# haoxiangsnr/Wave-U-Net-for-Speech-Enhancement

Measured on AMD Instinct MI355X. Metric: 16384-sample frames/sec fwd+bwd, 12-level Wave-U-Net, higher is better.
Workload: dtype f32 (levels >= 16 samples: 3 x f16 MFMA on hi/lo fp16 halves, fp32 accumulate; the rest f32 MFMA); 1 GPU; unet_basic 12-level, 16384-sample frames, batch=64 per GPU, fp32, training-mode forward + smooth_l1 + backward + fused HIP Adam step (BASELINE.json configs[2]; configs[3] when n_gpus>1); global_batch=64, frame=16384, parallelism=dp1

## Files before the change

### wave-u-net-for-speech-enhancement_amd/csrc/wunet_backward.cpp

```cpp
#include "wunet_host.h"
#include "wunet_elementwise.h"
#include "wunet_tiny.h"
#include "wunet_h3_elem.h"
#include "wunet_input_grad.h"

using namespace wunet_host;

namespace {
#ifndef WUNET_EMU
__global__ void stamp_kernel(unsigned long long* p) { *p = wall_clock64(); }
unsigned long long* g_stamps = nullptr;
bool stamps_on()
{
    static const bool on = getenv("WUNET_STAMP") != nullptr;
    if (on && !g_stamps && (hipMalloc(&g_stamps, 128 * sizeof(unsigned long long)) != hipSuccess || hipMemset(g_stamps, 0, 128 * sizeof(unsigned long long)) != hipSuccess)) g_stamps = nullptr;
    return on && g_stamps;
}
#define WUNET_STAMP(stream_, slot_) { if (stamps_on()) hipLaunchKernelGGL(stamp_kernel, dim3(1), dim3(1), 0, stream_, g_stamps + (slot_)); }
#else
#define WUNET_STAMP(stream_, slot_) {}
#endif

bool dx_stays_split(const wunet_ctx* c, int i)
{
// ... 259 lines not shown
    }
    return q.dx_sum ? sum_dx_splits(k, l) : WUNET_OK;
}

int weight_gradient(const BwdCall& k, int i, const BwdLayerPlan& q)
{
    wunet_ctx* c = k.c; float* ws = k.ws; const hipStream_t sd = k.sd;
    const int NL = c->NL;
    const LayerPlan& l = c->ly[i];
    if (sd != k.st && hipStreamWaitEvent(sd, k.side->ev_fork, 0) != hipSuccess) return fail(WUNET_E_RUNTIME, "fork onto the weight-gradient stream failed");
    WUNET_STAMP(sd, 2 * i + 1)
    if (i == NL - 1) {
        WUNET_LAUNCH(rows_sum_kernel, dim3(2), dim3(WUNET_THREADS), 0, sd,
                     (const float*)(ws + c->hpart_off), c->head_blocks, 2, k.grads[4 * NL] + c->ci, 1, k.grads[4 * NL + 1]);
        WUNET_CHECK_LAUNCH();
        WUNET_LAUNCH(rows_sum_kernel, dim3(c->ci), dim3(WUNET_THREADS), 0, sd,
                     (const float*)(ws + c->hpart2_off), l.a_split, c->ci, k.grads[4 * NL], c->ci, k.grads[4 * NL + 1]);
        WUNET_CHECK_LAUNCH();
    }
    if (q.e0) return WUNET_OK;
    const float* xin = i == 0 ? k.noisy : ws + l.xin;
    const size_t nw = (size_t)l.cout * l.cin * l.taps;
    if (q.tiny) {
        WUNET_LAUNCH(tiny_wgrad_kernel, dim3((unsigned)((nw + WUNET_THREADS - 1) / WUNET_THREADS)), dim3(WUNET_THREADS), 0, sd,
                     (const float*)(ws + l.g), xin, k.grads[4 * i], c->B, l.cin, l.cout, l.L, l.taps);
        WUNET_CHECK_LAUNCH();
        return WUNET_OK;
    }
    int rc;
    if (l.h3w)
        rc = launch_wgrad_h3(l, l.hw, reinterpret_cast<const wunet_half*>(ws + l.xh), reinterpret_cast<const wunet_half*>(ws + l.xl),
                             reinterpret_cast<const wunet_half*>(ws + l.gzh), reinterpret_cast<const wunet_half*>(ws + l.gzl),
                             gz_scale_slot(c, ws, i), x_scale_slot(c, ws, i),
                             ws + c->wgpart_off, c->B, sd, c->bf);
    else {
        WgradArgs w = make_wgrad_args(xin, ws + l.g, ws + c->wgpart_off, c->B, l.cin, l.cout, l.L, l.taps, l.w.cps);
        if (q.gz_in_wgrad) {
            w.z = ws + l.z; w.k1 = ws + l.k1; w.k2 = ws + l.k2; w.k3 = ws + l.k3; w.Lt = l.Lt;
        }
        rc = launch_wgrad_any(l.taps, w, l.w, sd);
    }
    if (rc) return rc;
    WUNET_CHECK_LAUNCH();
    if (l.h3w) {
        WgradH3ReduceArgs ra{};
        ra.part = ws + c->wgpart_off; ra.part_stride = h3w_part_stride(l, l.hw); ra.splits = l.hw.ksplit; ra.dw = k.grads[4 * i];
        ra.Cout = l.cout; ra.Cin = l.cin; ra.taps = l.taps; ra.mrep = l.hw.mrep; ra.tw = l.taps == 15 ? 8 : 5;
        ra.nblocks = l.hw.nblocks; ra.mblocks = l.hw.mblocks; ra.cib = l.taps == 15 ? 32 : 64;
        int serial_max = 64; long long serial_min_n4 = 8192;
#ifdef WUNET_EMU
        if (const char* e = getenv("WUNET_REDUCE_SERIAL")) sscanf(e, "%d,%lld", &serial_max, &serial_min_n4);
#endif
        const size_t n4 = ra.part_stride / 4;
        if (ra.splits <= serial_max && (long long)n4 >= serial_min_n4) {
            WUNET_LAUNCH(wgrad_h3_reduce_serial_kernel, dim3(capped_blocks(n4, WUNET_THREADS, 4096)), dim3(WUNET_THREADS), 0, sd, ra);
        } else {
            WUNET_LAUNCH(wgrad_h3_reduce_kernel, dim3(capped_blocks(n4, 16, 4096)), dim3(WUNET_THREADS), 0, sd, ra);
        }
    } else {
        const unsigned blocks = capped_blocks(nw / 4, 16, 4096);
        WUNET_LAUNCH(wgrad_reduce_kernel, dim3(blocks < 1 ? 1 : blocks), dim3(WUNET_THREADS), 0, sd,
                     (const float*)(ws + c->wgpart_off), l.w.rows, nw, k.grads[4 * i]);
    }
    WUNET_CHECK_LAUNCH();
    return WUNET_OK;
}

// ... 123 lines not shown
```

### wave-u-net-for-speech-enhancement_amd/csrc/wunet_h3.h

```cpp
#pragma once
#include "wunet_dev.h"

#ifdef WUNET_EMU
static const unsigned wunet_zero16[8] = {0, 0, 0, 0, 0, 0, 0, 0};
#else
static __device__ __attribute__((aligned(16))) const unsigned wunet_zero16[8] = {0, 0, 0, 0, 0, 0, 0, 0};
#endif

struct ConvH3Args {
    const wunet_half* xh; const wunet_half* xl;
    const wunet_half* wh; const wunet_half* wl;
    unsigned xdelta, wdelta;
    const void* zpad;
    const float* bias;
    const float* sc;
    const float* sc2;
    float* out;
    float* stats;
    const float* ev_a; const float* ev_s; float* xrows;
    unsigned long long* trace;
    int B, Cout, C8, NCH, L, logL;
    int NS, NFS;
    int ntiles, mblocks;
    int stages_per_split;
// ... 134 lines not shown
                {
                    const int krow = ((ks * 32) / LSEG) * SWX + (ks * 32) % LSEG;
                    const wunet_half* p = xs + xbase + (krow + OB + tw) * 8;
                    const wunet_h8 bh = wunet_ldtr8(p, p + 32);
                    wunet_h8 bl = bh;
                    if (!BF) bl = wunet_ldtr8(p + XG * XPOS * 8, p + XG * XPOS * 8 + 32);
#pragma unroll
                    for (int mt = 0; mt < M_REP; ++mt) {
                        if (BF) acc[mt][tw] = wunet_mfma16b(ah[mt], bh, acc[mt][tw]);
                        else {
                            acc[mt][tw] = wunet_mfma16h(al[mt], bh, acc[mt][tw]);
                            acc[mt][tw] = wunet_mfma16h(ah[mt], bl, acc[mt][tw]);
                            acc[mt][tw] = wunet_mfma16h(ah[mt], bh, acc[mt][tw]);
                        }
                    }
                }
            }
        }
    }
#undef WUNET_WH3_PREFETCH

    WUNET_WH3_STORE_PART(M_REP, TW, A, acc, blockIdx.x, (size_t)blockIdx.z * gridDim.y + blockIdx.y, wave, lane)
}

struct WgradH3dArgs {
    const wunet_half* xh; const wunet_half* xl;
    const wunet_half* gh; const wunet_half* gl;
    const float* sc;
    const float* sc2;
    float* part;
    int B, Cin, Cout, XC8, GC8, L, logL, chunks_per_split;
    size_t part_stride;
    int cin_active;
    int xcd_walk, ksplit, nblocks, mblocks;
};

template <int TAPS, int M_REP, bool DB, bool BF = false, int TP = 128>
__global__ __launch_bounds__(WUNET_THREADS, ((DB && TP == 128) ? 1 : 2)) void wgrad_h3d_kernel(WgradH3dArgs A)
{
    constexpr int GP = TP + 4, XPOS = TP + 20;
    static_assert(TP == 128 || TP == 64, "chunk");
    constexpr int WG = TAPS == 15 ? 2 : 4;
    constexpr int TW = TAPS == 15 ? 8 : 5;
    constexpr int OB = TAPS == 15 ? 1 : 8 - TAPS / 2;
    constexpr int CIB = WG * 16, XG = CIB / 8, GG = M_REP * 2;
    constexpr int NPL = BF ? 1 : 2;
    constexpr int GPCS = NPL * GG * GP;
    constexpr int XPCS = NPL * XG * XPOS;
    constexpr int GIT = (GPCS + WUNET_THREADS - 1) / WUNET_THREADS;
    constexpr int XIT = (XPCS + WUNET_THREADS - 1) / WUNET_THREADS;
    constexpr int BUF = (GPCS + XPCS + 8) * 8;
    WUNET_DYN_SMEM(smem);
    wunet_half* lds = reinterpret_cast<wunet_half*>(smem);

    const int tid = threadIdx.x, lane = tid & 63, wave = tid >> 6, q = lane >> 4, i16 = lane & 15;
    const int grp = TAPS == 15 ? wave >> 1 : wave;
    const int t0 = TAPS == 15 ? (wave & 1) * 8 : 0;
    int bx = blockIdx.x, by = blockIdx.y, bz = blockIdx.z;
    if (A.xcd_walk) {
        const int nyz = A.nblocks * A.mblocks;
        const int grp8 = (int)blockIdx.x / (8 * nyz), rem = (int)blockIdx.x - grp8 * 8 * nyz;
        const int yz = rem >> 3;
        bx = grp8 * 8 + (rem & 7); by = yz % A.nblocks; bz = yz / A.nblocks;
        if (bx >= A.ksplit) return;
    }
    const int co0 = bz * M_REP * 16, ci0 = by * CIB;
    const int L = A.L;
    const long long nchunks = ((long long)A.B * L) / TP;
    const long long kbeg = (long long)bx * A.chunks_per_split;
    long long kend = kbeg + A.chunks_per_split;
    if (kend > nchunks) kend = nchunks;

    const int tr_row = (i16 >> 2) + q * 8, tr_pl = (i16 & 3) >> 1, tr_h = (i16 & 1) * 4;
    const int gbase = (tr_pl * GP + tr_row) * 8 + tr_h;
    const int xbase = GPCS * 8 + ((grp * 2 + tr_pl) * XPOS + tr_row + t0) * 8 + tr_h;

    long long gsrc[GIT]; int gsel[GIT];
    long long xsrc[XIT]; int xrow[XIT], xsel[XIT];
#pragma unroll
    for (int it = 0; it < GIT; ++it) {
        const int f = tid + it * WUNET_THREADS;
        const int pl = f / GP, r = f - pl * GP;
        const int c8 = (co0 >> 3) + (pl % GG);
        gsel[it] = (f < GPCS && r < TP) ? ((c8 < A.GC8 ? 1 : 0) | (pl >= GG ? 2 : 0)) : -1;
        gsrc[it] = ((long long)c8 * L + r) * 8;
    }
#pragma unroll
    for (int it = 0; it < XIT; ++it) {
        const int f = tid + it * WUNET_THREADS;
        const int pl = f / XPOS, r = f - pl * XPOS;
        const int c8 = (ci0 >> 3) + (pl % XG);
        xsel[it] = f < XPCS ? ((c8 < A.XC8 ? 1 : 0) | (pl >= XG ? 2 : 0)) : -1;
        xrow[it] = r - 8;
        xsrc[it] = ((long long)c8 * L + (r - 8)) * 8;
    }
    const wunet_half* const zero_ = reinterpret_cast<const wunet_half*>(wunet_zero16);
#define WUNET_WH3D_DMA(K_, BUF_)                                                                                  \
    {                                                                                                             \
        const long long n0_ = (K_) * TP;                                                                          \
        const int b_ = (int)(n0_ >> A.logL), l0_ = (int)(n0_ & (L - 1));                                          \
        wunet_half* dst_ = lds + (size_t)(BUF_) * BUF + (size_t)wave * 64 * 8;                                    \
        _Pragma("unroll") for (int it = 0; it < GIT; ++it) {                                                      \
            if (gsel[it] >= 0) {                                                                                  \
                const wunet_half* src_ = (gsel[it] & 2) ? A.gl : A.gh;                                            \
                const wunet_half* p_ = (gsel[it] & 1) ? src_ + (size_t)b_ * A.GC8 * L * 8 + gsrc[it] + (size_t)l0_ * 8 : zero_; \
                wunet_dma16(p_, dst_ + (size_t)it * WUNET_THREADS * 8);                                           \
            }                                                                                                     \
        }                                                                                                         \
        _Pragma("unroll") for (int it = 0; it < XIT; ++it) {                                                      \
            if (xsel[it] >= 0) {                                                                                  \
                const int l_ = l0_ + xrow[it];                                                                    \
                const wunet_half* src_ = (xsel[it] & 2) ? A.xl : A.xh;                                            \
                const wunet_half* p_ = ((xsel[it] & 1) && l_ >= 0 && l_ < L)                                      \
                                           ? src_ + (size_t)b_ * A.XC8 * L * 8 + xsrc[it] + (size_t)l0_ * 8 : zero_; \
                wunet_dma16(p_, dst_ + (size_t)GPCS * 8 + (size_t)it * WUNET_THREADS * 8);                        \
            }                                                                                                     \
        }                                                                                                         \
    }

    wunet_f4 acc[M_REP][TW];
#pragma unroll
    for (int mt = 0; mt < M_REP; ++mt)
#pragma unroll
        for (int tw = 0; tw < TW; ++tw) acc[mt][tw] = wunet_f4{0.f, 0.f, 0.f, 0.f};

    const bool active = wunet_uniform(ci0 + grp * 16 < A.cin_active ? 1 : 0) != 0;
    if (DB && kbeg < kend) WUNET_WH3D_DMA(kbeg, 0)
    for (long long k = kbeg; k < kend; ++k) {
        const int cur = DB ? (int)((k - kbeg) & 1) : 0;
        if (!DB) {
            __syncthreads();
            WUNET_WH3D_DMA(k, 0)
        }
        wunet_dma_wait();
        __syncthreads();
        if (DB && k + 1 < kend) WUNET_WH3D_DMA(k + 1, cur ^ 1)
        const wunet_half* gs = lds + (size_t)cur * BUF;
        constexpr int KS = TP / 32;
        if (!active) continue;
        wunet_h8 ah[2][M_REP], al[2][M_REP], bh[2], bl[2];
#define WUNET_WH3D_LOAD_A(BUF_, KS_)                                                                              \
    _Pragma("unroll") for (int mt = 0; mt < M_REP; ++mt) {                                                        \
        const wunet_half* p = gs + gbase + ((mt * 2) * GP + (KS_) * 32) * 8;                                      \
        ah[BUF_][mt] = wunet_ldtr8(p, p + 32);                                                                    \
        if (!BF) al[BUF_][mt] = wunet_ldtr8(p + GG * GP * 8, p + GG * GP * 8 + 32);                               \
    }
#define WUNET_WH3D_LOAD_B(BUF_, KS_, TW_)                                                                         \
    {                                                                                                             \
        const wunet_half* p = gs + xbase + ((KS_) * 32 + OB + (TW_)) * 8;                                         \
        bh[BUF_] = wunet_ldtr8(p, p + 32);                                                                        \
        if (!BF) bl[BUF_] = wunet_ldtr8(p + XG * XPOS * 8, p + XG * XPOS * 8 + 32);                               \
    }
        WUNET_WH3D_LOAD_A(0, 0)
        WUNET_WH3D_LOAD_B(0, 0, 0)
#pragma unroll
        for (int ks = 0; ks < KS; ++ks) {
#pragma unroll
            for (int tw = 0; tw < TW; ++tw) {
                const int sb = (ks * TW + tw) & 1, ab = ks & 1;
                if (tw + 1 < TW) {
                    if (sb) { WUNET_WH3D_LOAD_B(0, ks, tw + 1) } else { WUNET_WH3D_LOAD_B(1, ks, tw + 1) }
                } else if (ks + 1 < KS) {
                    if (ab) { WUNET_WH3D_LOAD_A(0, ks + 1) } else { WUNET_WH3D_LOAD_A(1, ks + 1) }
                    if (sb) { WUNET_WH3D_LOAD_B(0, ks + 1, 0) } else { WUNET_WH3D_LOAD_B(1, ks + 1, 0) }
                }
                wunet_sched_fence();
                if (BF) {
#pragma unroll
                    for (int mt = 0; mt < M_REP; ++mt) acc[mt][tw] = wunet_mfma16b(ah[ab][mt], bh[sb], acc[mt][tw]);
                } else {
#pragma unroll
                    for (int mt = 0; mt < M_REP; ++mt) acc[mt][tw] = wunet_mfma16h(al[ab][mt], bh[sb], acc[mt][tw]);
#pragma unroll
                    for (int mt = 0; mt < M_REP; ++mt) acc[mt][tw] = wunet_mfma16h(ah[ab][mt], bl[sb], acc[mt][tw]);
#pragma unroll
                    for (int mt = 0; mt < M_REP; ++mt) acc[mt][tw] = wunet_mfma16h(ah[ab][mt], bh[sb], acc[mt][tw]);
                }
            }
        }
#undef WUNET_WH3D_LOAD_A
#undef WUNET_WH3D_LOAD_B
    }
#undef WUNET_WH3D_DMA

    WUNET_WH3_STORE_PART(M_REP, TW, A, acc, bx, (size_t)bz * (A.xcd_walk ? (unsigned)A.nblocks : gridDim.y) + by, wave, lane)
}
```

### wave-u-net-for-speech-enhancement_amd/csrc/wunet_host.h

```cpp
#pragma once
#include <cstdarg>
#include <cmath>
#include <cstdio>
#include <cstdlib>
#include <cstring>
#include <map>
#include <mutex>
#include <string>
#include <vector>

#include "wunet_kernels.h"
#include "wunet_h3.h"
#include "wunet_h3u.h"
#include "wunet_launch.h"
#include "wunet_hip.h"

namespace wunet_host {

int fail(int code, const char* fmt, ...);
const char* last_error_text();

#define WUNET_CHECK_LAUNCH()                                                                   \
    do {                                                                                       \
        hipError_t e_ = hipGetLastError();                                                     \
        if (e_ != hipSuccess) return wunet_host::fail(WUNET_E_RUNTIME, "%s:%d HIP error: %s", __FILE__, __LINE__, hipGetErrorString(e_)); \
    } while (0)

extern bool g_prof_on;
void prof_begin(hipStream_t st, const char* name, double flops, double bytes);
void prof_end(hipStream_t st);
long long prof_collect(char* buf, size_t cap);
extern unsigned long long* g_h3_trace;

inline int ilog2(long long v) { int r = 0; while ((1LL << r) < v) ++r; return r; }
inline bool is_pow2(long long v) { return v > 0 && (v & (v - 1)) == 0; }
inline size_t align64(size_t v) { return (v + 63) & ~(size_t)63; }
inline int round_up(int v, int m) { return (v + m - 1) / m * m; }
inline unsigned capped_blocks(size_t n, size_t per_block, size_t cap) { const size_t b = (n + per_block - 1) / per_block; return (unsigned)(b < cap ? b : cap); }
inline int kc_of(int taps) { return taps == 15 ? 4 : 12; }

struct ConvCfg { int mrep, nrep, mtiles_p, mblocks, cp, grid_x, ksplit, kcps; };
ConvCfg plan_conv(int B, int L, int rows, int kch, int taps);
ConvArgs make_conv_args(const float* x, int kch, const float* wpk, const float* bias, float* out, float* stats,
                        int B, int rows, int L, int taps, const ConvCfg& c, size_t split_stride);
int launch_conv(int taps, const ConvArgs& a, const ConvCfg& c, hipStream_t st);

struct WgradCfg { int mrep, nw, xit, wsplit, mblocks, nblocks, ksplit, cps, rows; };
WgradCfg plan_wgrad(int B, int L, int cin, int cout, int taps);
WgradArgs make_wgrad_args(const float* x, const float* g, float* part, int B, int Cin, int Cout, int L, int taps, int cps);
int launch_wgrad_any(int taps, const WgradArgs& a, const WgradCfg& w, hipStream_t st);

enum { LK_RAW = 0, LK_DECIM = 1, LK_UPCAT = 2 };

struct PlanSwitches {
    const char *order_f, *order_d, *order_w;
    bool no_split, old_split, ktail_off, no_skip_fuse, no_evop, no_e0, upt_off, wgrad_xcd_off;
    int sps, h3u_eval, h3u_train, a_cap;
};
PlanSwitches read_plan_switches();

struct H3ConvPlan { int mrep, mtp, nch, sps, ksplit, ntiles, ntt; };
H3ConvPlan plan_h3_conv(int B, int L, int rows, int kch, int taps, bool transposed, int bf, const PlanSwitches& sw);
struct H3WgradPlan { int mrep, mblocks, nblocks, ksplit, cps, tp, xcd, dma, db; };
H3WgradPlan plan_h3_wgrad(int B, int L, int cin, int cout, int taps, int bf, const PlanSwitches& sw);

struct LayerGeom {
    int cin, cout, taps, L, logL, kind;
    int Lt;
    int src0, src1;
    int c0;
};
struct LayerDecisions {
    ConvCfg f;
    ConvCfg d;
    WgradCfg w;
    int f_rows;
    int a_split;
    size_t f_wpk, d_wpk;
    size_t z, a, s, mean, rstd, xin, g, dx, k1, k2, k3;
    size_t wl1;
    int evop;
    int h3f, h3d, h3w;
    H3ConvPlan hf, hd;
    H3WgradPlan hw;
    int first;
    int h3x;
    int skip_from;
    int h3u, h3u_train;
    int feeds_h3;
    size_t xh, xl, xzp;
    size_t gzh, gzl, gzp;
    size_t h3f_wpk, h3d_wpk;
    int upt;
    size_t dxh, usp;
};
struct LayerPlan : LayerGeom, LayerDecisions {};

size_t h3d_smem(int nseg, int mrep, int bf, int mtp, int eval, int upt = 0);
int h3d_blocks_per_cu(int nseg, int mrep, int bf);
int h3_stage_count(int kch, int taps, int ntt);
size_t h3w_part_stride(const LayerGeom& g, const H3WgradPlan& w);
size_t h3w_dma_smem(const LayerGeom& g, const H3WgradPlan& w, int bf);
bool up_pairs_regular(int Lin);
unsigned pack_gx();

}

struct wunet_ctx {
    int n, ci, B, T, NL;
    int Tt = 0;
    bool padded = false;
    size_t pad_in = 0, pad_out = 0, pad_gout = 0;
    std::vector<wunet_host::LayerPlan> ly;
    size_t stats_off, wpkf_off, spart_off, fwd_floats;
    size_t bmax_off, bound_off;
    size_t bpart_off, wgpart_off, wpkb_off, gh_off, hpart_off, hpart2_off, e0part_off, total_floats;
    int e0 = 1;
    int head_blocks;
    int h3 = 0;
    int bf = 0;
    std::vector<unsigned char> frozen;
    bool any_frozen = false;
    size_t h3_wf_hi, h3_wf_lo, h3_wb_hi, h3_wb_lo, h3_slot;
    size_t fslot_off, wmax_off;
    size_t h3_wf_halfs, h3_wb_halfs;
    struct Side {
        hipStream_t stream = nullptr; hipEvent_t ev_fork = nullptr, ev_join = nullptr, ev_pack = nullptr, ev_fpack = nullptr, ev_fpack2 = nullptr;
        const void* packed_ws = nullptr;
    };
    std::map<int, Side> side;
    std::mutex side_lock;
};

namespace wunet_host {

void layout_workspace(wunet_ctx* c);
int launch_split(const float* x, wunet_half* hi, wunet_half* lo, const float* sc, const float* xb0, const float* xb1, float* xsc,
                 int B, int C, int L, hipStream_t st, int bf = 0);
float* x_scale_slot(const wunet_ctx* c, float* ws, int layer);
float* w_scale_slot(const wunet_ctx* c, float* ws, int layer);
float* act_bound_slot(const wunet_ctx* c, float* ws, int layer);
float* gz_scale_slot(const wunet_ctx* c, float* ws, int layer);
struct ConvH3OpOut { wunet_half* h; wunet_half* l; const float* wl1; const float* xmax; float* xsc; int C8; };
struct ConvH3Upt { int c0; float up_scale; float* uh_out; float* uh_spill; };
struct ConvH3Launch {
    int taps, mrep, mtiles_p, sps, nch, ntt;
    int B, rows, kch, L, bf;
    const wunet_half *xh, *xl, *wh, *wl;
    const void* zpad;
    const float *bias, *sc, *sc2;
    float *out, *stats;
    const float *ev_a, *ev_s; float* xrows;
    const ConvH3OpOut* op;
    const ConvH3Upt* upt;
};
int launch_conv_h3(const ConvH3Launch& k, hipStream_t st);
int launch_conv_h3u(const ConvH3uArgs& a, int mrep, int mtiles_p, int kch, hipStream_t st);
int launch_wgrad_h3(const LayerGeom& g, const H3WgradPlan& w, const wunet_half* xh, const wunet_half* xl, const wunet_half* gh, const wunet_half* gl,
                    const float* sc, const float* sc2, float* part, int B, hipStream_t st, int bf = 0);
int launch_backward_packs(wunet_ctx* c, const float* const* params, float* ws, hipStream_t st);
wunet_ctx::Side* side_for_current_device(wunet_ctx* c);
bool side_stream_off();

}
```

### wave-u-net-for-speech-enhancement_amd/csrc/wunet_launchers.cpp

```cpp
#include "wunet_host.h"
#include "wunet_elementwise.h"
#include "wunet_h3_elem.h"

namespace wunet_host {

ConvArgs make_conv_args(const float* x, int kch, const float* wpk, const float* bias, float* out, float* stats,
                        int B, int rows, int L, int taps, const ConvCfg& c, size_t split_stride)
{
    ConvArgs a{};
    a.x = x; a.wpk = wpk; a.bias = bias; a.out = out; a.stats = stats;
    a.B = B; a.Cin = kch; a.Cout = rows; a.CinP = c.cp; a.L = L; a.logL = ilog2(L);
    const int tn = 64 * c.nrep;
    a.seg = L < tn ? L : tn;
    a.seg_shift = ilog2(a.seg);
    a.segw = a.seg + 16;
    const int rowlen = (tn / a.seg) * a.segw;
    int rp = rowlen;
    while (rp % 32 != 16) rp += 4;
    a.rowp = rp;
    a.r4 = rowlen / 4;
    a.sw4 = a.segw / 4;
    a.r4_magic = (unsigned)(((1u << 20) + a.r4 - 1) / a.r4);
    a.sw4_magic = (unsigned)(((1u << 20) + a.sw4 - 1) / a.sw4);
    a.kc_per_split = c.kcps;
// ... 121 lines not shown
    if (gx < nitems) gx &= ~7;
    if (gx < 8) gx = 8;
    if (gx > nitems) gx = nitems;
    const dim3 grid((unsigned)gx, (unsigned)ksplit);
    const int rc = wunet_launch_conv_h3d(a, taps, mrep, nseg, grid, smem, st, bf != 0, op != nullptr, upt != nullptr);
    prof_end(st);
    if (rc != 0) return fail(WUNET_E_ARG, "no conv_h3 kernel for taps=%d mrep=%d nseg=%d (rc %d)", taps, mrep, nseg, rc);
    return 0;
}

int launch_conv_h3u(const ConvH3uArgs& a0, int mrep, int mtiles_p, int kch, hipStream_t st)
{
    ConvH3uArgs a = a0;
    const double posn = (double)a.B * a.L;
    a.logL = ilog2(a.L);
    a.C8 = (kch + 7) / 8;
    a.NS = (a.C8 + 3) / 4;
    a.ntiles = (int)((posn + 255) / 256); a.mblocks = mtiles_p / mrep;
    a.trace = g_h3_trace ? g_h3_trace + (1 << 20) : nullptr;
    const size_t smem = (size_t)(2 * 2 * 4 * 272 + 2 * 2 * mrep * 5 * 64) * 16 + (size_t)(WUNET_WAVES * mrep * 32 + 4 + 2 * a.C8 * 8 + 3 * mtiles_p * 16) * sizeof(float);
    const int nitems = a.ntiles * a.mblocks;
    int gx = h3_grid_cap() / 2;
    if (gx > nitems) gx = nitems;
    char pname[64];
    snprintf(pname, sizeof pname, "conv_h3u_kernel<%d>", mrep);
    prof_begin(st, pname, 2.0 * posn * a.Cout * kch * 5.0, 4.0 * posn * (a.Cout + a.C0 * 0.5 + a.C1));
    const int rc = wunet_launch_conv_h3u(a, mrep, dim3((unsigned)gx), smem, st);
    prof_end(st);
    if (rc != 0) return fail(WUNET_E_ARG, "no conv_h3u kernel for mrep=%d (rc %d)", mrep, rc);
    return 0;
}

int launch_wgrad_h3(const LayerGeom& l, const H3WgradPlan& w, const wunet_half* xh, const wunet_half* xl, const wunet_half* gh, const wunet_half* gl,
                    const float* sc, const float* sc2, float* part, int B, hipStream_t st, int bf)
{
    char pname[96];
    const double posn = (double)B * l.L;
    const int xg = l.taps == 15 ? 4 : 8, tp = w.tp, nseg = l.L >= tp ? 1 : tp / l.L;
    const dim3 grid(w.ksplit, w.nblocks, w.mblocks);
    const int npl = bf ? 1 : 2;
    int rc;
    const auto fill = [&](auto& a) {
        a.xh = xh; a.xl = xl; a.gh = gh; a.gl = gl; a.sc = sc; a.sc2 = sc2; a.part = part; a.B = B; a.Cin = l.cin; a.Cout = l.cout;
        a.XC8 = (l.cin + 7) / 8; a.GC8 = (l.cout + 7) / 8; a.L = l.L; a.logL = l.logL;
        a.chunks_per_split = w.cps; a.part_stride = h3w_part_stride(l, w);
    };
    snprintf(pname, sizeof pname, "wgrad_h3%s_kernel<%d, %d%s>", w.dma ? "d" : "", l.taps, w.mrep, bf ? ", bf16" : "");
    prof_begin(st, pname, 2.0 * posn * l.cout * l.cin * l.taps, 4.0 * posn * (l.cout + l.cin));
    if (w.dma) {
        WgradH3dArgs a{};
        fill(a);
        a.cin_active = l.cin;
        a.ksplit = w.ksplit; a.nblocks = w.nblocks; a.mblocks = w.mblocks;
        a.xcd_walk = w.xcd;
        const size_t smem_d = h3w_dma_smem(l, w, bf);
        const int nyz = w.nblocks * w.mblocks;
        const dim3 grid_x((unsigned)(((w.ksplit + 7) / 8) * 8 * nyz));
        rc = wunet_launch_wgrad_h3d(a, l.taps, w.mrep, w.db != 0, a.xcd_walk ? grid_x : grid, w.db ? smem_d : smem_d / 2, st, bf != 0, tp);
    } else {
        WgradH3Args a{};
        fill(a);
        const int xrows = nseg == 1 ? tp + 20 : nseg * (tp / nseg + 16), xpos = ((xrows + 11) / 16) * 16 + 4;
        const size_t smem = ((size_t)npl * (w.mrep * 2) * (tp + 4) + (size_t)npl * xg * xpos + 8) * 16;
        rc = wunet_launch_wgrad_h3(a, l.taps, w.mrep, nseg, tp, grid, smem, st, bf != 0);
    }
    prof_end(st);
    if (rc != 0) return fail(WUNET_E_ARG, "no wgrad_h3 kernel for taps=%d mrep=%d (rc %d)", l.taps, w.mrep, rc);
    return 0;
}

int launch_backward_packs(wunet_ctx* c, const float* const* params, float* ws, hipStream_t st)
{
    const int NL = c->NL;
    PackTable tab{};
    int nd = 0;
    for (int i = 1; i < NL; ++i) {
        const LayerPlan& l = c->ly[i];
        if (l.h3d) continue;
        PackDesc& d = tab.d[nd++];
        d.w = params[4 * i]; d.dst = ws + c->wpkb_off + l.d_wpk;
        d.Cout = l.cout; d.Cin = l.cin; d.taps = l.taps; d.M = l.cin; d.CP = l.d.cp; d.mtiles = l.d.mtiles_p; d.transposed = 1;
    }
    if (nd > 0) {
        WUNET_LAUNCH(pack_weights_kernel, dim3(pack_gx(), nd), dim3(WUNET_THREADS), 0, st, tab);
        WUNET_CHECK_LAUNCH();
// ... 54 lines not shown
```

### wave-u-net-for-speech-enhancement_amd/csrc/wunet_ops.cpp

```cpp
#include "wunet_host.h"
#include "wunet_elementwise.h"
#include "wunet_h3_elem.h"
#include "wunet_loss_rows.h"
#include "wunet_stft.h"
#include "wunet_stoi.h"
#include "wunet_mix.h"
#include "wunet_reverb.h"

using namespace wunet_host;

extern "C" {

size_t wunet_loss_scratch_bytes(void) { return 256 * sizeof(double); }

int wunet_loss_forward(int kind, const float* clean, const float* enhanced, size_t n, float* loss_out, void* scratch, void* stream)
{
    if (kind < 0 || kind > 2 || !clean || !enhanced || !loss_out || !scratch || n == 0) return fail(WUNET_E_ARG, "bad loss argument");
    hipStream_t st = (hipStream_t)stream;
    const unsigned blocks = capped_blocks(n, WUNET_THREADS * 8, 256);
    WUNET_LAUNCH(loss_partial_kernel, dim3(blocks), dim3(WUNET_THREADS), 0, st, kind, clean, enhanced, n, (double*)scratch);
    WUNET_CHECK_LAUNCH();
    WUNET_LAUNCH(loss_final_kernel, dim3(1), dim3(WUNET_THREADS), 0, st, (const double*)scratch, (int)blocks, n, loss_out);
    WUNET_CHECK_LAUNCH();
    return WUNET_OK;
// ... 825 lines not shown
    ConvH3Launch h{};
    h.taps = K; h.mrep = p.mrep; h.mtiles_p = p.mtp; h.sps = p.sps; h.nch = p.nch; h.ntt = p.ntt;
    h.B = B; h.rows = rows; h.kch = kch; h.L = L;
    h.xh = xs.h(); h.xl = xs.l(); h.zpad = xs.zpad(); h.wh = whp; h.wl = wlp;
    h.bias = split ? nullptr : bias; h.sc = xslot; h.sc2 = wslot + 2; h.out = split ? part.f() : out;
    rc = launch_conv_h3(h, st);
    if (!rc && split) {
        const unsigned blocks = capped_blocks(nout, WUNET_THREADS, 2048);
        const float* partp = part.f();
        const int ks = p.ksplit;
        WUNET_LAUNCH(split_sum_kernel, dim3(blocks), dim3(WUNET_THREADS), 0, st, partp, ks, nout, out, bias, rows, ilog2(L));
    }
    hipStreamSynchronize(st);
    if (rc) return rc;
    WUNET_CHECK_LAUNCH();
    return WUNET_OK;
}
}

int wunet_op_conv1d_split(const float* x, const float* w, const float* bias, float* z, int B, int Cin, int Cout, int L, int K, void* stream)
{
    if (op_split_check(B, Cin, Cout, L, K, false)) return WUNET_E_ARG;
    return op_conv_split_common(x, w, bias, z, B, Cin, Cout, Cout, Cin, L, K, 0, (hipStream_t)stream);
}

int wunet_op_conv1d_dgrad_split(const float* gz, const float* w, float* dx, int B, int Cin, int Cout, int L, int K, void* stream)
{
    if (op_split_check(B, Cin, Cout, L, K, true)) return WUNET_E_ARG;
    return op_conv_split_common(gz, w, nullptr, dx, B, Cout, Cin, Cout, Cin, L, K, 1, (hipStream_t)stream);
}

int wunet_op_conv1d_wgrad_split(const float* gz, const float* x, float* dw, int B, int Cin, int Cout, int L, int K, void* stream)
{
    if (op_split_check(B, Cin, Cout, L, K, true)) return WUNET_E_ARG;
    hipStream_t st = (hipStream_t)stream;
    LayerGeom l{};
    l.cin = Cin; l.cout = Cout; l.taps = K; l.L = L; l.logL = ilog2(L);
    const H3WgradPlan w = plan_h3_wgrad(B, L, Cin, Cout, K, 0, read_plan_switches());
    SplitBuf xs, gs;
    DevBuf misc, part;
    const int cmax = Cin > Cout ? Cin : Cout;
    if (!misc.alloc((16 + 2 * (size_t)cmax) * sizeof(float)) || !part.alloc((size_t)w.ksplit * h3w_part_stride(l, w) * sizeof(float)))
        return fail(WUNET_E_RUNTIME, "hipMalloc");
    float* gslot = misc.f(), *xslot = misc.f() + 8, *oz = misc.f() + 16;
    WUNET_LAUNCH(fill_kernel, dim3(4), dim3(WUNET_THREADS), 0, st, oz, (size_t)cmax, 1.0f);
    WUNET_LAUNCH(fill_kernel, dim3(4), dim3(WUNET_THREADS), 0, st, oz + cmax, (size_t)cmax, 0.0f);
    int rc = op_split_operand(gz, B, Cout, L, gs, gslot, oz, oz + cmax, st);
    if (!rc) rc = op_split_operand(x, B, Cin, L, xs, xslot, oz, oz + cmax, st);
    if (!rc) rc = launch_wgrad_h3(l, w, xs.h(), xs.l(), gs.h(), gs.l(), gslot, xslot, part.f(), B, st);
    if (!rc) {
        WgradH3ReduceArgs ra{};
        ra.part = part.f(); ra.part_stride = h3w_part_stride(l, w); ra.splits = w.ksplit; ra.dw = dw;
        ra.Cout = Cout; ra.Cin = Cin; ra.taps = K; ra.mrep = w.mrep; ra.tw = K == 15 ? 8 : 5;
        ra.nblocks = w.nblocks; ra.mblocks = w.mblocks; ra.cib = K == 15 ? 32 : 64;
        WUNET_LAUNCH(wgrad_h3_reduce_kernel, dim3(capped_blocks(ra.part_stride / 4, 16, 4096)), dim3(WUNET_THREADS), 0, st, ra);
    }
    hipStreamSynchronize(st);
    if (rc) return rc;
    WUNET_CHECK_LAUNCH();
    return WUNET_OK;
}

}
```

### wave-u-net-for-speech-enhancement_amd/csrc/wunet_plan.cpp

```cpp
#include <algorithm>
#include "wunet_host.h"
#include "wunet_h3_elem.h"

namespace wunet_host {

namespace { thread_local std::string g_err; }

int fail(int code, const char* fmt, ...)
{
    char buf[512];
    va_list ap;
    va_start(ap, fmt);
    vsnprintf(buf, sizeof buf, fmt, ap);
    va_end(ap);
    g_err = buf;
    return code;
}

const char* last_error_text() { return g_err.c_str(); }

namespace {
struct ProfRec { std::string name; double flops; double bytes; hipEvent_t e0, e1; };
std::vector<ProfRec> g_prof;
}
// ... 151 lines not shown
        const int occ_lds = (int)(160 * 1024 / lds);
        if (occ_lds < occ) occ = occ_lds < 1 ? 1 : occ_lds;
        const long long slots = 256LL * occ;
        const long long mn = (long long)w.mblocks * w.nblocks;
        long long ks = slots / mn;
        if (ks < 1) ks = 1;
        if (ks > chunks) ks = chunks;
        w.ksplit = (int)ks;
        w.cps = (int)((chunks + ks - 1) / ks);
        w.ksplit = (int)((chunks + w.cps - 1) / w.cps);
    }
    w.rows = w.ksplit * (w.wsplit ? 4 : 1);
    return w;
}
unsigned pack_gx() { return 512; }

PlanSwitches read_plan_switches()
{
    const auto is_zero = [](const char* name) { const char* e = getenv(name); return e != nullptr && atoi(e) == 0; };
    PlanSwitches sw{};
    sw.order_f = getenv("WUNET_H3_ORDER"); sw.order_d = getenv("WUNET_H3D_ORDER"); sw.order_w = getenv("WUNET_H3W_ORDER");
    sw.no_split = getenv("WUNET_H3_NOSPLIT") != nullptr; sw.old_split = getenv("WUNET_H3_OLDSPLIT") != nullptr;
    if (const char* e = getenv("WUNET_H3_SPS")) sw.sps = atoi(e);
    sw.ktail_off = is_zero("WUNET_H3_KTAIL");
    sw.h3u_eval = 512; sw.h3u_train = 2048;
    if (const char* e = getenv("WUNET_H3U")) {
        int a = 0, b = 0;
        const int got = sscanf(e, "%d,%d", &a, &b);
        if (got == 2) { sw.h3u_eval = a; sw.h3u_train = b; }
        else if (got == 1) sw.h3u_eval = sw.h3u_train = a;
    }
    sw.no_skip_fuse = getenv("WUNET_NO_SKIP_FUSE") != nullptr; sw.no_evop = getenv("WUNET_NO_EVOP") != nullptr; sw.no_e0 = getenv("WUNET_NO_E0") != nullptr;
    sw.upt_off = is_zero("WUNET_UPT"); sw.wgrad_xcd_off = is_zero("WUNET_WGRAD_XCD");
    sw.a_cap = getenv("WUNET_A_CAP") ? atoi(getenv("WUNET_A_CAP")) : 128;
    return sw;
}

int pick_mrep_h3(int mtiles, const char* ord)
{
    int best = 2, best_pad = 1 << 30;
    for (const char* p = ord; *p; ++p) {
        const int m = *p - '0';
        const int pad = round_up(mtiles, m) - mtiles;
        if (pad < best_pad) { best_pad = pad; best = m; }
    }
    return best;
}

const char* h3_order(int taps, int L, int ntiles, int mtiles)
{
    return (taps == 5 && L >= 256 && (long long)ntiles * ((mtiles + 3) / 4) >= 512) ? "432" : "32";
}

size_t h3w_part_stride(const LayerGeom& g, const H3WgradPlan& w)
{
    const int tw = g.taps == 15 ? 8 : 5;
    return (size_t)w.mblocks * w.nblocks * WUNET_WAVES * w.mrep * tw * 256;
}
size_t h3w_dma_smem(const LayerGeom& g, const H3WgradPlan& w, int bf)
{
    const int xg = g.taps == 15 ? 4 : 8, tp = w.tp, npl = bf ? 1 : 2;
    return (size_t)2 * (npl * (w.mrep * 2) * (tp + 4) + npl * xg * (tp + 20) + 8) * 16;
}
static bool h3w_regs_allow_two_blocks(int taps, int mrep) { return (taps == 5 && mrep <= 4) || (taps == 15 && mrep <= 3); }

size_t h3d_smem(int nseg, int mrep, int bf, int mtp, int eval, int upt)
// ... 125 lines not shown
        l.d = plan_conv(B, l.L, l.cin, l.cout, l.taps);
        l.w = plan_wgrad(B, l.L, l.cin, l.cout, l.taps);
        if (l.L < 4) { l.f.ksplit = 1; l.d.ksplit = 1; }
        l.first = (i == 0 && l.cin == 1 && l.taps == 15 && l.L >= 256) ? 1 : 0;
        const long long posn = (long long)B * l.L;
        const bool big = c->h3 && !l.first && l.L >= 16 && posn >= 256 &&
                         (c->h3 == 2 || (l.L >= 256 ? (l.f.nrep == 4 && l.f.ksplit == 1) : posn >= 1024));
        l.h3f = big ? 1 : 0;
        l.h3d = (big && i > 0 && l.cin >= 16 && (c->h3 == 2 || l.L < 256 || (l.d.nrep == 4 && l.d.ksplit == 1))) ? 1 : 0;
        l.h3w = l.h3d;
        l.h3x = l.h3w;
        if (l.h3f) {
            l.hf = plan_h3_conv(B, l.L, l.cout, l.cin, l.taps, false, c->bf, sw);
            l.f.ksplit = l.hf.ksplit;
            l.f.grid_x = l.hf.ntiles;
        }
        if (l.h3d) {
            l.hd = plan_h3_conv(B, l.L, l.cin, l.cout, l.taps, true, c->bf, sw);
            l.d.ksplit = l.hd.ksplit;
        }
        if (l.h3w) l.hw = plan_h3_wgrad(B, l.L, l.cin, l.cout, l.taps, c->bf, sw);
        if (l.first) { l.f.ksplit = 1; l.f.grid_x = (int)(((long long)B * l.L + 1023) / 1024); }
        const bool can = h3u_can_run(c, l);
        l.h3u = (can && sw.h3u_eval > 0 && l.L >= sw.h3u_eval) ? 1 : 0;
        l.h3u_train = (can && sw.h3u_train > 0 && l.L >= sw.h3u_train) ? 1 : 0;
        l.f_rows = l.h3f ? l.f.grid_x : l.f.grid_x * WUNET_WAVES;
        const long long sp = posn / 4096;
        const int a_cap = sw.a_cap < 1 ? 1 : (sw.a_cap > 256 ? 256 : sw.a_cap);
        l.a_split = (int)(sp < 1 ? 1 : (sp > a_cap ? a_cap : sp));
    }
    const long long hb = ((long long)B * c->T) / 2048;
    c->head_blocks = (int)(hb < 1 ? 1 : (hb > 1024 ? 1024 : hb));
    c->e0 = sw.no_e0 ? 0 : 1;
}

static bool skip_planned(const LayerPlan& e, const LayerPlan& d) { return e.kind == LK_DECIM && d.kind == LK_UPCAT && e.h3x && d.h3x && d.src1 == e.src0 && d.c0 % 8 == 0; }
static bool evop_planned(const wunet_ctx* c, const LayerPlan& p, const LayerPlan& q, int pi)
{
    return p.h3f && !p.first && p.taps == 15 && p.L >= 256 && p.f.ksplit == 1 && p.hf.mrep <= 4 && q.kind == LK_DECIM && q.src0 == pi && q.h3f && q.h3x &&
           !c->bf && !c->padded;
}
static bool upt_planned(const wunet_ctx* c, const LayerPlan& q, const LayerPlan& p)
{
    return q.kind == LK_UPCAT && q.h3d && q.L >= 256 && q.d.ksplit == 1 && !(q.c0 & 3) && !(q.cin & 3) && q.c0 == p.cout && !c->bf && !c->padded &&
           p.h3d && p.L >= 128 && up_pairs_regular(q.L / 2);
}
static void plan_handoffs(wunet_ctx* c, const PlanSwitches& sw)
{
    for (int i = 1; i <= c->n && !sw.no_skip_fuse; ++i) {
        LayerPlan& d = c->ly[2 * c->n - i + 1];
        if (skip_planned(c->ly[i], d)) d.skip_from = i;
    }
    for (int i = 1; i + 1 <= c->n && !sw.no_evop; ++i)
        if (evop_planned(c, c->ly[i], c->ly[i + 1], i)) c->ly[i].evop = 1;
    for (int i = 1; i < c->NL; ++i) {
        const LayerPlan& l = c->ly[i];
        if (!l.h3f) continue;
        c->ly[l.src0].feeds_h3 = 1;
        if (l.kind == LK_UPCAT) c->ly[l.src1].feeds_h3 = 1;
    }
    for (int i = c->n + 1; i < c->NL && !sw.upt_off; ++i)
        if (upt_planned(c, c->ly[i], c->ly[c->ly[i].src0])) c->ly[i].upt = 1;
}

struct Bump { size_t off; size_t take(size_t floats) { const size_t at = off; off += align64(floats); return at; } };

// ... 192 lines not shown
```

Baseline: 12920 frames/s.

## Share K-slices across idle waves in h3 wgrad when few Cin groups are active

When a wgrad block has only a fraction of its Cin groups active (small Cin), the idle waves previously skipped compute. The kernel now splits the chunk's K-steps across those spare waves, then reduces their partial accumulators through LDS into the owning wave before storing the partial. This puts otherwise idle waves to work on narrow layers, at the cost of extra LDS handoff traffic and barriers per m-tile. An env switch can disable it, and the op entry's argument check is loosened.

```diff
diff --git a/wave-u-net-for-speech-enhancement_amd/csrc/wunet_backward.cpp b/wave-u-net-for-speech-enhancement_amd/csrc/wunet_backward.cpp
--- a/wave-u-net-for-speech-enhancement_amd/csrc/wunet_backward.cpp
+++ b/wave-u-net-for-speech-enhancement_amd/csrc/wunet_backward.cpp
@@ -315,7 +315,7 @@
         rc = launch_wgrad_h3(l, l.hw, reinterpret_cast<const wunet_half*>(ws + l.xh), reinterpret_cast<const wunet_half*>(ws + l.xl),
                              reinterpret_cast<const wunet_half*>(ws + l.gzh), reinterpret_cast<const wunet_half*>(ws + l.gzl),
                              gz_scale_slot(c, ws, i), x_scale_slot(c, ws, i),
-                             ws + c->wgpart_off, c->B, sd, c->bf);
+                             ws + c->wgpart_off, c->B, sd, c->bf, c->h3w_noshare);
     else {
         WgradArgs w = make_wgrad_args(xin, ws + l.g, ws + c->wgpart_off, c->B, l.cin, l.cout, l.L, l.taps, l.w.cps);
         if (q.gz_in_wgrad) {
diff --git a/wave-u-net-for-speech-enhancement_amd/csrc/wunet_h3.h b/wave-u-net-for-speech-enhancement_amd/csrc/wunet_h3.h
--- a/wave-u-net-for-speech-enhancement_amd/csrc/wunet_h3.h
+++ b/wave-u-net-for-speech-enhancement_amd/csrc/wunet_h3.h
@@ -190,6 +190,7 @@
     int B, Cin, Cout, XC8, GC8, L, logL, chunks_per_split;
     size_t part_stride;
     int cin_active;
+    int noshare;
     int xcd_walk, ksplit, nblocks, mblocks;
 };
 
@@ -214,6 +215,10 @@
     const int tid = threadIdx.x, lane = tid & 63, wave = tid >> 6, q = lane >> 4, i16 = lane & 15;
     const int grp = TAPS == 15 ? wave >> 1 : wave;
     const int t0 = TAPS == 15 ? (wave & 1) * 8 : 0;
+    constexpr int KS = TP / 32;
+    constexpr bool SHARE = !BF && !(TAPS == 5 && !DB && M_REP >= 3);
+    constexpr int SLOTS = TAPS == 15 ? 2 : 3;
+    static_assert((size_t)SLOTS * TW * 256 * sizeof(float) <= (size_t)BUF * sizeof(wunet_half), "hand-over of one m-tile inside one staging buffer");
     int bx = blockIdx.x, by = blockIdx.y, bz = blockIdx.z;
     if (A.xcd_walk) {
         const int nyz = A.nblocks * A.mblocks;
@@ -231,26 +236,28 @@
 
     const int tr_row = (i16 >> 2) + q * 8, tr_pl = (i16 & 3) >> 1, tr_h = (i16 & 1) * 4;
     const int gbase = (tr_pl * GP + tr_row) * 8 + tr_h;
+    const int crem = A.cin_active - ci0;
+    const int nact = crem >= CIB ? WG : (crem <= 0 ? 0 : (crem + 15) >> 4);
+    const bool share = SHARE && A.noshare == 0 && nact >= 1 && 2 * nact <= WG;
     const int xbase = GPCS * 8 + ((grp * 2 + tr_pl) * XPOS + tr_row + t0) * 8 + tr_h;
 
-    long long gsrc[GIT]; int gsel[GIT];
-    long long xsrc[XIT]; int xrow[XIT], xsel[XIT];
-#pragma unroll
-    for (int it = 0; it < GIT; ++it) {
-        const int f = tid + it * WUNET_THREADS;
-        const int pl = f / GP, r = f - pl * GP;
-        const int c8 = (co0 >> 3) + (pl % GG);
-        gsel[it] = (f < GPCS && r < TP) ? ((c8 < A.GC8 ? 1 : 0) | (pl >= GG ? 2 : 0)) : -1;
-        gsrc[it] = ((long long)c8 * L + r) * 8;
-    }
-#pragma unroll
-    for (int it = 0; it < XIT; ++it) {
-        const int f = tid + it * WUNET_THREADS;
-        const int pl = f / XPOS, r = f - pl * XPOS;
-        const int c8 = (ci0 >> 3) + (pl % XG);
-        xsel[it] = f < XPCS ? ((c8 < A.XC8 ? 1 : 0) | (pl >= XG ? 2 : 0)) : -1;
-        xrow[it] = r - 8;
-        xsrc[it] = ((long long)c8 * L + (r - 8)) * 8;
+#define WUNET_WH3D_PIECES(TID_)                                                                                   \
+    long long gsrc[GIT]; int gsel[GIT];                                                                           \
+    long long xsrc[XIT]; int xrow[XIT], xsel[XIT];                                                                \
+    _Pragma("unroll") for (int it = 0; it < GIT; ++it) {                                                          \
+        const int f = (TID_) + it * WUNET_THREADS;                                                                \
+        const int pl = f / GP, r = f - pl * GP;                                                                   \
+        const int c8 = (co0 >> 3) + (pl % GG);                                                                    \
+        gsel[it] = (f < GPCS && r < TP) ? ((c8 < A.GC8 ? 1 : 0) | (pl >= GG ? 2 : 0)) : -1;        \
+        gsrc[it] = ((long long)c8 * L + r) * 8;                                                                   \
+    }                                                                                                             \
+    _Pragma("unroll") for (int it = 0; it < XIT; ++it) {                                                          \
+        const int f = (TID_) + it * WUNET_THREADS;                                                                \
+        const int pl = f / XPOS, r = f - pl * XPOS;                                                               \
+        const int c8 = (ci0 >> 3) + (pl % XG);                                                                    \
+        xsel[it] = f < XPCS ? ((c8 < A.XC8 ? 1 : 0) | (pl >= XG ? 2 : 0)) : -1;                                   \
+        xrow[it] = r - 8;                                                                                         \
+        xsrc[it] = ((long long)c8 * L + (r - 8)) * 8;                                                             \
     }
     const wunet_half* const zero_ = reinterpret_cast<const wunet_half*>(wunet_zero16);
 #define WUNET_WH3D_DMA(K_, BUF_)                                                                                  \
@@ -282,21 +289,16 @@
 #pragma unroll
         for (int tw = 0; tw < TW; ++tw) acc[mt][tw] = wunet_f4{0.f, 0.f, 0.f, 0.f};
 
-    const bool active = wunet_uniform(ci0 + grp * 16 < A.cin_active ? 1 : 0) != 0;
-    if (DB && kbeg < kend) WUNET_WH3D_DMA(kbeg, 0)
-    for (long long k = kbeg; k < kend; ++k) {
-        const int cur = DB ? (int)((k - kbeg) & 1) : 0;
-        if (!DB) {
-            __syncthreads();
-            WUNET_WH3D_DMA(k, 0)
-        }
-        wunet_dma_wait();
-        __syncthreads();
-        if (DB && k + 1 < kend) WUNET_WH3D_DMA(k + 1, cur ^ 1)
-        const wunet_half* gs = lds + (size_t)cur * BUF;
-        constexpr int KS = TP / 32;
-        if (!active) continue;
-        wunet_h8 ah[2][M_REP], al[2][M_REP], bh[2], bl[2];
+#define WUNET_WH3D_STAGE(K_)                                                                                      \
+    const int cur = DB ? (int)(((K_) - kbeg) & 1) : 0;                                                            \
+    if (!DB) {                                                                                                    \
+        __syncthreads();                                                                                          \
+        WUNET_WH3D_DMA(K_, 0)                                                                                     \
+    }                                                                                                             \
+    wunet_dma_wait();                                                                                             \
+    __syncthreads();                                                                                              \
+    if (DB && (K_) + 1 < kend) WUNET_WH3D_DMA((K_) + 1, cur ^ 1)                                                  \
+    const wunet_half* gs = lds + (size_t)cur * BUF;
 #define WUNET_WH3D_LOAD_A(BUF_, KS_)                                                                              \
     _Pragma("unroll") for (int mt = 0; mt < M_REP; ++mt) {                                                        \
         const wunet_half* p = gs + gbase + ((mt * 2) * GP + (KS_) * 32) * 8;                                      \
@@ -309,6 +311,81 @@
         bh[BUF_] = wunet_ldtr8(p, p + 32);                                                                        \
         if (!BF) bl[BUF_] = wunet_ldtr8(p + XG * XPOS * 8, p + XG * XPOS * 8 + 32);                               \
     }
+#define WUNET_WH3D_MMA(AB_, SB_, TW_)                                                                             \
+    if (BF) {                                                                                                     \
+        _Pragma("unroll") for (int mt = 0; mt < M_REP; ++mt) acc[mt][TW_] = wunet_mfma16b(ah[AB_][mt], bh[SB_], acc[mt][TW_]); \
+    } else {                                                                                                      \
+        _Pragma("unroll") for (int mt = 0; mt < M_REP; ++mt) acc[mt][TW_] = wunet_mfma16h(al[AB_][mt], bh[SB_], acc[mt][TW_]); \
+        _Pragma("unroll") for (int mt = 0; mt < M_REP; ++mt) acc[mt][TW_] = wunet_mfma16h(ah[AB_][mt], bl[SB_], acc[mt][TW_]); \
+        _Pragma("unroll") for (int mt = 0; mt < M_REP; ++mt) acc[mt][TW_] = wunet_mfma16h(ah[AB_][mt], bh[SB_], acc[mt][TW_]); \
+    }
+
+    if (SHARE && share) {
+        const int nown = TAPS == 15 ? 2 : nact;
+        const int nsh = (WG >> (nact - 1)) < KS ? (WG >> (nact - 1)) : KS;
+        const int sh = wunet_uniform(wave >> (nown >> 1)), ownw = wave & (nown - 1);
+        const int egrp = TAPS == 15 ? 0 : ownw;
+        int tid_s = tid;
+        wunet_opaque(tid_s);
+        WUNET_WH3D_PIECES(tid_s)
+        const int xbase = GPCS * 8 + ((egrp * 2 + tr_pl) * XPOS + tr_row + t0) * 8 + tr_h;
+        if (DB && kbeg < kend) WUNET_WH3D_DMA(kbeg, 0)
+        for (long long k = kbeg; k < kend; ++k) {
+            WUNET_WH3D_STAGE(k)
+            wunet_h8 ah[1][M_REP], al[1][M_REP], bh[2], bl[2];
+            const wunet_half* const chunk = gs;
+#pragma unroll 1
+            for (int ks = sh; ks < KS; ks += nsh) {
+                int krow = ks * 32 * 8;
+                wunet_opaque(krow);
+                const wunet_half* gs = chunk + krow;
+                WUNET_WH3D_LOAD_A(0, 0)
+                WUNET_WH3D_LOAD_B(0, 0, 0)
+#pragma unroll
+                for (int tw = 0; tw < TW; ++tw) {
+                    if (tw + 1 < TW) {
+                        if (tw & 1) { WUNET_WH3D_LOAD_B(0, 0, tw + 1) } else { WUNET_WH3D_LOAD_B(1, 0, tw + 1) }
+                    }
+                    wunet_sched_fence();
+                    WUNET_WH3D_MMA(0, tw & 1, tw)
+                }
+            }
+        }
+        float* hand = reinterpret_cast<float*>(smem) + lane * 4;
+#pragma unroll
+        for (int mt = 0; mt < M_REP; ++mt) {
+            __syncthreads();
+            if (sh > 0 && sh < nsh) {
+#pragma unroll
+                for (int tw = 0; tw < TW; ++tw) {
+                    wunet_st4(hand + (((sh - 1) * nown + ownw) * TW + tw) * 256, acc[mt][tw]);
+                    acc[mt][tw] = wunet_f4{0.f, 0.f, 0.f, 0.f};
+                }
+            }
+            __syncthreads();
+            if (sh == 0) {
+#pragma unroll 1
+                for (int h = 1; h < nsh; ++h) {
+#pragma unroll
+                    for (int tw = 0; tw < TW; ++tw) {
+                        const wunet_f4 v = wunet_ld4(hand + (((h - 1) * nown + wave) * TW + tw) * 256);
+#pragma unroll
+                        for (int r = 0; r < 4; ++r) acc[mt][tw][r] += v[r];
+                    }
+                }
+            }
+        }
+        WUNET_WH3_STORE_PART(M_REP, TW, A, acc, bx, (size_t)bz * (A.xcd_walk ? (unsigned)A.nblocks : gridDim.y) + by, wave, lane)
+        return;
+    }
+
+    const bool active = wunet_uniform(ci0 + grp * 16 < A.cin_active ? 1 : 0) != 0;
+    WUNET_WH3D_PIECES(tid)
+    if (DB && kbeg < kend) WUNET_WH3D_DMA(kbeg, 0)
+    for (long long k = kbeg; k < kend; ++k) {
+        WUNET_WH3D_STAGE(k)
+        if (!active) continue;
+        wunet_h8 ah[2][M_REP], al[2][M_REP], bh[2], bl[2];
         WUNET_WH3D_LOAD_A(0, 0)
         WUNET_WH3D_LOAD_B(0, 0, 0)
 #pragma unroll
@@ -323,22 +400,15 @@
                     if (sb) { WUNET_WH3D_LOAD_B(0, ks + 1, 0) } else { WUNET_WH3D_LOAD_B(1, ks + 1, 0) }
                 }
                 wunet_sched_fence();
-                if (BF) {
-#pragma unroll
-                    for (int mt = 0; mt < M_REP; ++mt) acc[mt][tw] = wunet_mfma16b(ah[ab][mt], bh[sb], acc[mt][tw]);
-                } else {
-#pragma unroll
-                    for (int mt = 0; mt < M_REP; ++mt) acc[mt][tw] = wunet_mfma16h(al[ab][mt], bh[sb], acc[mt][tw]);
-#pragma unroll
-                    for (int mt = 0; mt < M_REP; ++mt) acc[mt][tw] = wunet_mfma16h(ah[ab][mt], bl[sb], acc[mt][tw]);
-#pragma unroll
-                    for (int mt = 0; mt < M_REP; ++mt) acc[mt][tw] = wunet_mfma16h(ah[ab][mt], bh[sb], acc[mt][tw]);
-                }
-            }
-        }
+                WUNET_WH3D_MMA(ab, sb, tw)
+            }
+        }
+    }
+#undef WUNET_WH3D_PIECES
+#undef WUNET_WH3D_STAGE
 #undef WUNET_WH3D_LOAD_A
 #undef WUNET_WH3D_LOAD_B
-    }
+#undef WUNET_WH3D_MMA
 #undef WUNET_WH3D_DMA
 
     WUNET_WH3_STORE_PART(M_REP, TW, A, acc, bx, (size_t)bz * (A.xcd_walk ? (unsigned)A.nblocks : gridDim.y) + by, wave, lane)
diff --git a/wave-u-net-for-speech-enhancement_amd/csrc/wunet_host.h b/wave-u-net-for-speech-enhancement_amd/csrc/wunet_host.h
--- a/wave-u-net-for-speech-enhancement_amd/csrc/wunet_host.h
+++ b/wave-u-net-for-speech-enhancement_amd/csrc/wunet_host.h
@@ -54,7 +54,7 @@
 
 struct PlanSwitches {
     const char *order_f, *order_d, *order_w;
-    bool no_split, old_split, ktail_off, no_skip_fuse, no_evop, no_e0, upt_off, wgrad_xcd_off;
+    bool no_split, old_split, ktail_off, no_skip_fuse, no_evop, no_e0, upt_off, wgrad_xcd_off, h3w_noshare;
     int sps, h3u_eval, h3u_train, a_cap;
 };
 PlanSwitches read_plan_switches();
@@ -115,6 +115,7 @@
     size_t stats_off, wpkf_off, spart_off, fwd_floats;
     size_t bmax_off, bound_off;
     size_t bpart_off, wgpart_off, wpkb_off, gh_off, hpart_off, hpart2_off, e0part_off, total_floats;
+    int h3w_noshare = 0;
     int e0 = 1;
     int head_blocks;
     int h3 = 0;
@@ -157,7 +158,7 @@
 int launch_conv_h3(const ConvH3Launch& k, hipStream_t st);
 int launch_conv_h3u(const ConvH3uArgs& a, int mrep, int mtiles_p, int kch, hipStream_t st);
 int launch_wgrad_h3(const LayerGeom& g, const H3WgradPlan& w, const wunet_half* xh, const wunet_half* xl, const wunet_half* gh, const wunet_half* gl,
-                    const float* sc, const float* sc2, float* part, int B, hipStream_t st, int bf = 0);
+                    const float* sc, const float* sc2, float* part, int B, hipStream_t st, int bf = 0, int noshare = 0);
 int launch_backward_packs(wunet_ctx* c, const float* const* params, float* ws, hipStream_t st);
 wunet_ctx::Side* side_for_current_device(wunet_ctx* c);
 bool side_stream_off();
diff --git a/wave-u-net-for-speech-enhancement_amd/csrc/wunet_launchers.cpp b/wave-u-net-for-speech-enhancement_amd/csrc/wunet_launchers.cpp
--- a/wave-u-net-for-speech-enhancement_amd/csrc/wunet_launchers.cpp
+++ b/wave-u-net-for-speech-enhancement_amd/csrc/wunet_launchers.cpp
@@ -177,7 +177,7 @@
 }
 
 int launch_wgrad_h3(const LayerGeom& l, const H3WgradPlan& w, const wunet_half* xh, const wunet_half* xl, const wunet_half* gh, const wunet_half* gl,
-                    const float* sc, const float* sc2, float* part, int B, hipStream_t st, int bf)
+                    const float* sc, const float* sc2, float* part, int B, hipStream_t st, int bf, int noshare)
 {
     char pname[96];
     const double posn = (double)B * l.L;
@@ -196,6 +196,7 @@
         WgradH3dArgs a{};
         fill(a);
         a.cin_active = l.cin;
+        a.noshare = noshare;
         a.ksplit = w.ksplit; a.nblocks = w.nblocks; a.mblocks = w.mblocks;
         a.xcd_walk = w.xcd;
         const size_t smem_d = h3w_dma_smem(l, w, bf);
diff --git a/wave-u-net-for-speech-enhancement_amd/csrc/wunet_ops.cpp b/wave-u-net-for-speech-enhancement_amd/csrc/wunet_ops.cpp
--- a/wave-u-net-for-speech-enhancement_amd/csrc/wunet_ops.cpp
+++ b/wave-u-net-for-speech-enhancement_amd/csrc/wunet_ops.cpp
@@ -881,11 +881,13 @@
 
 int wunet_op_conv1d_wgrad_split(const float* gz, const float* x, float* dw, int B, int Cin, int Cout, int L, int K, void* stream)
 {
-    if (op_split_check(B, Cin, Cout, L, K, true)) return WUNET_E_ARG;
+    if (op_check(B, Cin, Cout, L, K)) return WUNET_E_ARG;
+    if (L < 16 || (long long)B * L < 128 || Cin < 8) return fail(WUNET_E_ARG, "the split weight gradient needs L >= 16, B*L >= 128 and Cin >= 8");
     hipStream_t st = (hipStream_t)stream;
     LayerGeom l{};
     l.cin = Cin; l.cout = Cout; l.taps = K; l.L = L; l.logL = ilog2(L);
-    const H3WgradPlan w = plan_h3_wgrad(B, L, Cin, Cout, K, 0, read_plan_switches());
+    const PlanSwitches sw = read_plan_switches();
+    const H3WgradPlan w = plan_h3_wgrad(B, L, Cin, Cout, K, 0, sw);
     SplitBuf xs, gs;
     DevBuf misc, part;
     const int cmax = Cin > Cout ? Cin : Cout;
@@ -896,7 +898,7 @@
     WUNET_LAUNCH(fill_kernel, dim3(4), dim3(WUNET_THREADS), 0, st, oz + cmax, (size_t)cmax, 0.0f);
     int rc = op_split_operand(gz, B, Cout, L, gs, gslot, oz, oz + cmax, st);
     if (!rc) rc = op_split_operand(x, B, Cin, L, xs, xslot, oz, oz + cmax, st);
-    if (!rc) rc = launch_wgrad_h3(l, w, xs.h(), xs.l(), gs.h(), gs.l(), gslot, xslot, part.f(), B, st);
+    if (!rc) rc = launch_wgrad_h3(l, w, xs.h(), xs.l(), gs.h(), gs.l(), gslot, xslot, part.f(), B, st, 0, sw.h3w_noshare ? 1 : 0);
     if (!rc) {
         WgradH3ReduceArgs ra{};
         ra.part = part.f(); ra.part_stride = h3w_part_stride(l, w); ra.splits = w.ksplit; ra.dw = dw;
diff --git a/wave-u-net-for-speech-enhancement_amd/csrc/wunet_plan.cpp b/wave-u-net-for-speech-enhancement_amd/csrc/wunet_plan.cpp
--- a/wave-u-net-for-speech-enhancement_amd/csrc/wunet_plan.cpp
+++ b/wave-u-net-for-speech-enhancement_amd/csrc/wunet_plan.cpp
@@ -207,6 +207,7 @@
     }
     sw.no_skip_fuse = getenv("WUNET_NO_SKIP_FUSE") != nullptr; sw.no_evop = getenv("WUNET_NO_EVOP") != nullptr; sw.no_e0 = getenv("WUNET_NO_E0") != nullptr;
     sw.upt_off = is_zero("WUNET_UPT"); sw.wgrad_xcd_off = is_zero("WUNET_WGRAD_XCD");
+    if (const char* e = getenv("WUNET_H3W_NOSHARE")) sw.h3w_noshare = atoi(e) != 0;
     sw.a_cap = getenv("WUNET_A_CAP") ? atoi(getenv("WUNET_A_CAP")) : 128;
     return sw;
 }
@@ -398,6 +399,7 @@
     const long long hb = ((long long)B * c->T) / 2048;
     c->head_blocks = (int)(hb < 1 ? 1 : (hb > 1024 ? 1024 : hb));
     c->e0 = sw.no_e0 ? 0 : 1;
+    c->h3w_noshare = sw.h3w_noshare ? 1 : 0;
 }
 
 static bool skip_planned(const LayerPlan& e, const LayerPlan& d) { return e.kind == LK_DECIM && d.kind == LK_UPCAT && e.h3x && d.h3x && d.src1 == e.src0 && d.c0 % 8 == 0; }
```

Result: no change. 13040 frames/s, median of 6 (+0.9%).
